# phtryll/subword-tokenizers

Hardware: AMD Instinct MI355X
Metric: FastBPE encode MB/s (value; tokens bit-exact) + BPE train s/1k-merges (train.s_per_1k_merges) (higher is better)
Workload: dtype u32; 1 GPU; configs[1]: FastBPE encode, S85k-open stand-in for train-85k (85,000 sentences, 8.53 MB/GPU), first 8,000 pretrained merges -- the slower of S85k-lex / S85k-open; sentences_per_gpu=85000, bytes_per_gpu=8526871, parallelism=corpus-sharded x1, no collective

## Files before the change

subword-tokenizers_amd/_build.py:

```python
import hashlib
import os
import shutil
import subprocess

_HERE = os.path.dirname(os.path.abspath(__file__))
CSRC = os.path.join(_HERE, "csrc")
LIB_DIR = os.path.join(_HERE, "_lib")
LIB_PATH = os.path.join(LIB_DIR, "libswt_hip.so")
SOURCES = ["swt_core.hip", "swt_tile.hip", "swt_dedup.hip", "swt_bpe_encode.hip", "swt_wp.hip", "swt_words.hip", "swt_bpe_train.hip", "swt_dist.hip", "swt_lower.hip", "swt_metrics.hip"]
HEADERS = ["swt_common.h", "swt_tile.h", "swt_dedup.h", "swt_words.h", "swt_train.h", "unicode_classes.inc", "unicode_lower.inc", os.path.join("..", "..", "include", "swt.h")]
FLAGS = ["--offload-arch=gfx950", "-O3", "-std=c++17", "-fPIC", "-Wall", "-Wno-unused-function"]
FLAGS += os.environ.get("SWT_EXTRA_FLAGS", "").split()


def _hipcc():
    for cand in (os.environ.get("HIPCC"), shutil.which("hipcc"), "/opt/rocm/bin/hipcc"):
        if cand and os.path.exists(cand):
            return cand
    raise RuntimeError("hipcc not found: libswt_hip.so cannot be built (set HIPCC or install ROCm)")


def _stamp():
    h = hashlib.sha256()
    for f in SOURCES + HEADERS:
        with open(os.path.join(CSRC, f), "rb") as fh:
            h.update(fh.read())
    h.update(" ".join(FLAGS).encode())
    return h.hexdigest()


def build(force=False, verbose=False):
    os.makedirs(LIB_DIR, exist_ok=True)
    stamp_path = os.path.join(LIB_DIR, "build.stamp")
    stamp = _stamp()
    if not force and os.path.exists(LIB_PATH) and os.path.exists(stamp_path):
        with open(stamp_path) as f:
            if f.read().strip() == stamp:
                return LIB_PATH
    hipcc = _hipcc()
    objs = []
    procs = []
    for src in SOURCES:
        obj = os.path.join(LIB_DIR, src.replace(".hip", ".o"))
        objs.append(obj)
        cmd = [hipcc] + FLAGS + ["-c", os.path.join(CSRC, src), "-o", obj]
        if verbose:
            print(" ".join(cmd))
        procs.append((src, subprocess.Popen(cmd, stdout=subprocess.PIPE, stderr=subprocess.STDOUT, text=True)))
    for src, p in procs:
        out, _ = p.communicate()
        if p.returncode != 0:
            raise RuntimeError("hipcc failed on %s:\n%s" % (src, out))
        if verbose and out.strip():
            print(out)
    cmd = [hipcc, "--offload-arch=gfx950", "-shared", "-fPIC", "-o", LIB_PATH] + objs + ["-ldl"]
    r = subprocess.run(cmd, stdout=subprocess.PIPE, stderr=subprocess.STDOUT, text=True)
    if r.returncode != 0:
        raise RuntimeError("link failed:\n" + r.stdout)
    with open(stamp_path, "w") as f:
        f.write(stamp)
    return LIB_PATH


# ... 31 lines not shown
```

subword-tokenizers_amd/csrc/swt_bpe_encode.hip:

```cpp
#include <cstring>
#include <unordered_map>
#include <utility>

#include "swt_dedup.h"
#include "swt_tile.h"
#include "swt_words.h"

namespace swt {

struct alignas(16) BpeSlot {
  uint64_t key;
  uint32_t rank;
  uint32_t merged;
};

constexpr uint8_t kClsWs = 1, kClsPunct = 2;
constexpr uint32_t kNoRank = 0xFFFFFFFFu;
#ifndef SWT_LANE_TILE
#define SWT_LANE_TILE 384
#endif
#ifndef SWT_LANE_CAP
#define SWT_LANE_CAP 512
#endif
constexpr int kLaneTile = SWT_LANE_TILE;
constexpr int kLaneCap = SWT_LANE_CAP;
constexpr uint64_t kDirectBytes = 1024, kDirectSents = 64;

struct BpeHash { uint32_t a, b, c; };
constexpr BpeHash kHash1{0x9E3779u, 0x85EBCBu, 0xC2B2AFu}, kHash2{0x27D4EBu, 0x165667u, 0x9E3779u};
__host__ __device__ __forceinline__ uint32_t bpe_hash(uint32_t l, uint32_t r, uint32_t sh, BpeHash k) {
  uint32_t x = (l & 0xFFFFFFu) * k.a + (r & 0xFFFFFFu) * k.b;
  x ^= x >> 16;
  return ((x & 0xFFFFFFu) * k.c) >> sh;
}

__device__ __forceinline__ bool slot_lookup(const BpeSlot *__restrict__ slots, uint32_t sh, uint32_t l, uint32_t r,
                                            uint32_t &rank, uint32_t &merged) {
  const uint4 r1 = *reinterpret_cast<const uint4 *>(&slots[bpe_hash(l, r, sh, kHash1)]);
  const uint4 r2 = *reinterpret_cast<const uint4 *>(&slots[bpe_hash(l, r, sh, kHash2)]);
  const bool h1 = r1.x == r && r1.y == l, h2 = r2.x == r && r2.y == l;
  rank = h1 ? r1.z : r2.z;
  merged = h1 ? r1.w : r2.w;
  return h1 || h2;
}

__device__ __forceinline__ uint32_t slot_value(const BpeSlot *__restrict__ slots, uint32_t sh, uint32_t l, uint32_t r) {
  const uint4 r1 = *reinterpret_cast<const uint4 *>(&slots[bpe_hash(l, r, sh, kHash1)]);
  const uint4 r2 = *reinterpret_cast<const uint4 *>(&slots[bpe_hash(l, r, sh, kHash2)]);
  const uint32_t a = (r1.x == r && r1.y == l) ? r1.z : kNoRank;
  const uint32_t b = (r2.x == r && r2.y == l) ? r2.z : kNoRank;
  return a & b;
}

__device__ uint32_t merge_word(uint32_t *s, uint32_t n, const BpeSlot *__restrict__ slots, uint32_t sh) {
  while (n >= 2) {
    uint32_t best = 0xFFFFFFFFu, bm = 0, bl = 0, br = 0;
    uint32_t a = s[0];
    for (uint32_t i = 0; i + 1 < n; i++) {
      const uint32_t b = s[i + 1];
      uint32_t rk, mg;
      if (slot_lookup(slots, sh, a, b, rk, mg) && rk < best) { best = rk; bm = mg; bl = a; br = b; }
      a = b;
    }
    if (best == 0xFFFFFFFFu) break;
    uint32_t j = 0, i = 0;
    while (i < n) {
      const uint32_t x = s[i];
      if (i + 1 < n && x == bl && s[i + 1] == br) { s[j++] = bm; i += 2; }
      else { s[j++] = x; i++; }
    }
    n = j;
  }
  return n;
}

struct GiantResult { uint64_t end; uint32_t ntok; };

__device__ GiantResult giant_word(const uint8_t *__restrict__ text, uint64_t pos, uint64_t send,
                                  const uint8_t *__restrict__ cls_tab, const BpeSlot *__restrict__ slots, uint32_t sh,
                                  uint32_t *out) {
  GiantResult r{pos, 0};
  uint32_t n = 0;
  bool first = true;
  while (r.end < send) {
    const uint8_t b = text[r.end];
    int len = utf8_len(b);
    if (r.end + len > send) len = (int)(send - r.end);
    uint32_t cp = b;
    if (b >= 0x80 && len > 1) {
      cp = b & (0xFF >> (len + 1));
      for (int i = 1; i < len; i++) cp = (cp << 6) | (text[r.end + i] & 0x3F);
    }
    const uint8_t c = utf8_is_cont(b) ? kClsWs : ((cls_tab && cp < kNumCodePoints) ? cls_tab[cp] : (uint8_t)0);
    if (c & kClsWs) { if (first) r.end += len; break; }
    if (c & kClsPunct) { if (first) { out[n++] = cp; r.end += len; } break; }
    out[n++] = cp;
    r.end += len;
    first = false;
  }
  n = merge_word(out, n, slots, sh);
  for (uint32_t i = 1; i < n; i++) out[i] |= SWT_BPE_CONT;
  r.ntok = n;
  return r;
}

template <int Cap>
struct LaneLds {
  static constexpr int Blocks = Cap / 64;
  __attribute__((aligned(16))) uint8_t txt[Cap + 16];
  uint32_t sym[Cap + 4];
  uint32_t val[Cap + 4];
  uint16_t wl[Cap + 2];
  unsigned long long sbits[Blocks + 1];
  unsigned long long symmask[Blocks + 1];
  unsigned long long vmask[Blocks + 1];
  uint32_t sympre[Blocks + 1];
  uint32_t blkpre[Blocks + 1];
};
struct LaneShared {
  uint32_t cls2[64];
  GiantResult giant;
};

struct LaneTile {
  uint64_t s_lo, s_hi;
  uint64_t span_base, span_end;
  uint64_t s_next;
  uint64_t cb;
  uint32_t *tile_out;
  uint32_t run;
};
struct LaneChunk {
  uint64_t abase;
  uint32_t off0, staged, nblk;
  uint32_t ce;
  uint32_t nsym, nw;
  int cut;
  bool last, giant;
};

__device__ __forceinline__ void wave_sync() {
  __builtin_amdgcn_fence(__ATOMIC_RELEASE, "wavefront");
  __builtin_amdgcn_wave_barrier();
  __builtin_amdgcn_fence(__ATOMIC_ACQUIRE, "wavefront");
}

constexpr uint32_t kDirtyVal = 0xFFFFFFFEu;

template <bool Packed>
__device__ void slow_word(uint32_t *S, uint32_t *V, const uint32_t n0, const BpeSlot *__restrict__ slots, uint32_t sh,
                          const uint32_t *__restrict__ merged_of_rank) {
  uint32_t n = n0;
  for (;;) {
    uint32_t m = kNoRank;
    for (uint32_t i = 0; i + 1 < n; i++) m = min(m, V[i]);
    if (m == kNoRank) break;
    const uint32_t mg = Packed ? (SWT_SYM_BASE + (m & 0xFFFFu)) : merged_of_rank[m];
    uint32_t i = 0, j = 0;
    while (i < n) {
      const uint32_t vi = V[i];
      const bool take = i + 1 < n && vi == m;
      const uint32_t s = take ? mg : (S[i] & ~SWT_BPE_CONT);
      if (take && j) V[j - 1] = kDirtyVal;
      S[j] = j ? (s | SWT_BPE_CONT) : s;
      V[j] = take ? kDirtyVal : vi;
      i += take ? 2u : 1u;
      j++;
    }
    n = j;
    V[n - 1] = kNoRank;
    for (uint32_t k = 0; k + 1 < n; k++)
      if (V[k] == kDirtyVal) V[k] = slot_value(slots, sh, S[k] & ~SWT_BPE_CONT, S[k + 1] & ~SWT_BPE_CONT);
  }
  for (uint32_t k = n; k < n0; k++) S[k] = kInvalidTok;
}

__device__ __forceinline__ void lane_classes(LaneShared &L, const uint8_t *__restrict__ cls_tab, int lane) {
  uint32_t w = 0;
  if (cls_tab) {
    const uint4 v = reinterpret_cast<const uint4 *>(cls_tab)[lane];
    auto pk = [](uint32_t d) {
      uint32_t x = d & 0x03030303u;
      x = (x | (x >> 6)) & 0x000F000Fu;
      return (x | (x >> 12)) & 0xFFu;
    };
    w = pk(v.x) | (pk(v.y) << 8) | (pk(v.z) << 16) | (pk(v.w) << 24);
  }
  L.cls2[lane] = w;
}

template <int Cap>
__device__ __forceinline__ void lane_split(LaneLds<Cap> &L, const uint32_t *cls2, const uint8_t *__restrict__ text, uint64_t n_bytes,
                                           const uint64_t *__restrict__ sent_off, const uint8_t *__restrict__ cls_tab,
                                           const BpeSlot *__restrict__ slots, uint32_t sh, const LaneTile &T, LaneChunk &C, int lane) {
  constexpr int Blocks = Cap / 64;
  const unsigned long long lt = (1ull << lane) - 1ull;
  const unsigned long long le = (2ull << lane) - 1ull;
  const uint64_t abase = T.cb & ~15ull;
  const uint32_t off0 = (uint32_t)(T.cb - abase);
  const uint64_t avail = T.span_end - abase;
  const bool last = avail <= (uint64_t)Cap;
  const uint32_t staged = last ? (uint32_t)avail : (uint32_t)Cap;
  const uint32_t nblk = (staged + 63) >> 6;

  for (uint32_t c = lane * 16; c < staged; c += 64 * 16) {
    const uint64_t g = abase + c;
    if (g + 16 <= n_bytes && ((reinterpret_cast<uintptr_t>(text + g) & 15) == 0)) {
      *reinterpret_cast<uint4 *>(&L.txt[c]) = *reinterpret_cast<const uint4 *>(text + g);
    } else {
      for (int i = 0; i < 16; i++) L.txt[c + i] = (g + i < n_bytes) ? text[g + i] : (uint8_t)' ';
    }
  }
  if (lane <= Blocks) L.sbits[lane] = 0ull;
  wave_sync();
  for (uint64_t s = T.s_next + lane; s < T.s_hi; s += 64) {
    const uint64_t o = sent_off[s];
    if (o >= abase + staged) break;
    if (o >= T.cb) atomicOr(&L.sbits[(o - abase) >> 6], 1ull << ((o - abase) & 63));
  }
  wave_sync();

  uint32_t nsym = 0, nw = 0;
  bool prev_wb = true;
  bool pend_open = false;
  uint32_t pend_cp = 0;
  int cut = -1;
  for (uint32_t blk = 0; blk < nblk; blk++) {
    const uint32_t p = blk * 64 + lane;
    const bool inr = p >= off0 && p < staged;
    const uint8_t b = inr ? L.txt[p] : (uint8_t)' ';
    const bool lead = !utf8_is_cont(b);
    uint32_t cp = b;
    if (b >= 0xC0) {
      int len = utf8_len(b);
      if (p + len > staged) len = (int)(staged - p);
      if (len > 1) {
        cp = b & (0xFF >> (len + 1));
        for (int i = 1; i < len; i++) cp = (cp << 6) | (L.txt[p + i] & 0x3F);
      }
    }
    uint32_t c = kClsWs;
    if (inr && lead)
      c = cp < 1024u ? ((cls2[cp >> 4] >> ((cp & 15u) << 1)) & 3u) : ((cls_tab && cp < kNumCodePoints) ? (cls_tab[cp] & 3u) : 0u);
    const unsigned long long INR = __ballot(inr);
    const unsigned long long LEAD = __ballot(lead);
    const unsigned long long WSm = __ballot(lead && (c & kClsWs));
    const unsigned long long PNm = __ballot(lead && (c & kClsPunct));
    const unsigned long long CONT = ~LEAD;
    unsigned long long WB = WSm | PNm | ((prev_wb && (CONT & 1ull)) ? 1ull : 0ull);
    WB |= (WB << 1) & CONT;
    WB |= (WB << 1) & CONT;
    WB |= (WB << 1) & CONT;
    const unsigned long long SS = L.sbits[blk];
    const unsigned long long first_bit = blk == 0 ? (1ull << off0) : 0ull;
    const unsigned long long before = (WB << 1) | (prev_wb ? 1ull : 0ull) | SS | first_bit;
    const unsigned long long SYM = LEAD & ~WSm & INR;
    const unsigned long long WSTART = SYM & (PNm | before);
    {
      const unsigned long long CUT = LEAD & (WSm | PNm | SS) & __ballot(inr && p > off0 && p + 4 <= staged);
      if (CUT) cut = (int)(blk * 64 + 63 - __builtin_clzll(CUT));
    }
    const bool is_sym = (SYM >> lane) & 1ull;
    const bool wstart = (WSTART >> lane) & 1ull;
    const unsigned long long after = SYM & ~le;
    const uint32_t q = after ? (uint32_t)__builtin_ctzll(after) : 64u;
    const bool hasnext = is_sym && q < 64 && !((WSTART >> (q & 63)) & 1ull);
    const uint32_t f = SYM ? (uint32_t)__builtin_ctzll(SYM) : 64u;
    const bool joins = pend_open && f < 64 && !((WSTART >> (f & 63)) & 1ull);
    const uint32_t si = nsym + (uint32_t)__popcll(SYM & lt);
    const uint32_t cpn = __shfl(cp, (int)(q & 63));
    const bool jp = joins && lane == 63;
    const uint32_t cpf = __builtin_amdgcn_readlane(cp, (int)(f & 63));
    const bool want = hasnext || jp;
    uint32_t v = kNoRank;
    if (want) v = slot_value(slots, sh, jp ? pend_cp : cp, jp ? cpf : cpn);
    if (is_sym) {
      L.sym[si] = wstart ? cp : (cp | SWT_BPE_CONT);
      if (!hasnext) L.val[si] = kNoRank;
    }
    if (want) L.val[jp ? nsym - 1 : si] = v;
    if (wstart) L.wl[nw + (uint32_t)__popcll(WSTART & lt)] = (uint16_t)si;
    if (lane == 0) { L.symmask[blk] = SYM; L.sympre[blk] = nsym; }
    nw += (uint32_t)__popcll(WSTART);
    nsym += (uint32_t)__popcll(SYM);
    if (SYM) {
      const int li = 63 - __builtin_clzll(SYM);
      const unsigned long long tail = li == 63 ? 0ull : ~((2ull << li) - 1ull);
      pend_open = ((WSm | PNm | SS) & tail) == 0ull && !((PNm >> li) & 1ull);
      pend_cp = __builtin_amdgcn_readlane(cp, li);
    } else {
      pend_open = false;
    }
    prev_wb = (WB >> 63) & 1ull;
  }
  wave_sync();
  C.abase = abase;
  C.off0 = off0;
  C.staged = staged;
  C.nblk = nblk;
  C.ce = staged;
  C.nsym = nsym;
  C.nw = nw;
  C.cut = cut;
  C.last = last;
  C.giant = false;
}

template <int Cap, int Mode>
__device__ __forceinline__ void lane_chunk_end(LaneLds<Cap> &L, GiantResult &giant, const uint8_t *__restrict__ text, const uint64_t *__restrict__ sent_off,
                                               const uint8_t *__restrict__ cls_tab, const BpeSlot *__restrict__ slots, uint32_t sh,
                                               LaneTile &T, LaneChunk &C, int lane, uint32_t *__restrict__ sent_local,
                                               const uint32_t *__restrict__ uslot, unsigned long long *__restrict__ rec,
                                               unsigned long long *__restrict__ drec, const DirectOut &direct) {
  constexpr bool kDirect = Mode == 2, kRec = Mode == 1;
  if (!C.last) {
    if (C.cut < 0) {
      if (lane == 0) {
        uint64_t s = T.s_next;
        while (s < T.s_hi && sent_off[s] <= T.cb) s++;
        const uint64_t send = sent_off[s];
        giant = giant_word(text, T.cb, send, cls_tab, slots, sh, T.tile_out + T.run);
      }
      wave_sync();
      const GiantResult g = giant;
      uint32_t mine = 0;
      for (uint64_t s = T.s_next + lane; s < T.s_hi; s += 64) {
        if (sent_off[s] >= g.end) break;
        if (kDirect) direct.off[s] = T.run; else if (Mode == 0) sent_local[s] = T.run;
        if (kRec) {
          drec[s] = (unsigned long long)(T.span_base + T.run) | ((unsigned long long)g.ntok << 32);
          rec[uslot[s]] = (unsigned long long)s | ((unsigned long long)g.ntok << 32);
        }
        mine++;
      }
      for (int d = 32; d >= 1; d >>= 1) mine += __shfl_xor(mine, d);
      T.s_next += mine;
      T.run += g.ntok;
      T.cb = g.end;
      C.giant = true;
      C.nw = 0;
      C.nsym = 0;
      wave_sync();
      return;
    }
    C.ce = (uint32_t)C.cut;
    C.nsym = L.sympre[C.ce >> 6] + (uint32_t)__popcll(L.symmask[C.ce >> 6] & ((1ull << (C.ce & 63)) - 1ull));
    uint32_t keep = 0;
    for (uint32_t k0 = 0; k0 < C.nw; k0 += 64) {
      const uint32_t k = k0 + lane;
      keep += (uint32_t)__popcll(__ballot(k < C.nw && L.wl[k] < C.nsym));
    }
    C.nw = keep;
  }
  if (lane == 0) L.wl[C.nw] = (uint16_t)C.nsym;
  T.cb = C.abase + C.ce;
  wave_sync();
}

template <int Cap>
__device__ __forceinline__ void lane_words_count(const LaneLds<Cap> &L, uint32_t nw, int lane, uint32_t &c2, uint32_t &c1, uint32_t &c0) {
  c0 = c1 = c2 = 0;
  for (uint32_t k0 = 0; k0 < nw; k0 += 64) {
    const uint32_t k = k0 + lane;
    const uint32_t n = k < nw ? (uint32_t)L.wl[k + 1] - (uint32_t)L.wl[k] : 0u;
    c0 += (uint32_t)__popcll(__ballot(n >= 2 && n <= 4));
    c1 += (uint32_t)__popcll(__ballot(n >= 5 && n <= 8));
    c2 += (uint32_t)__popcll(__ballot(n >= 9));
  }
}
template <int Cap>
__device__ __forceinline__ void lane_words_write(const LaneLds<Cap> &L, uint32_t nw, int lane, uint16_t *list, uint32_t o2, uint32_t o1,
                                                 uint32_t o0) {
  const unsigned long long lt = (1ull << lane) - 1ull;
  for (uint32_t k0 = 0; k0 < nw; k0 += 64) {
    const uint32_t k = k0 + lane;
    const uint32_t n = k < nw ? (uint32_t)L.wl[k + 1] - (uint32_t)L.wl[k] : 0u;
    const unsigned long long M0 = __ballot(n >= 2 && n <= 4), M1 = __ballot(n >= 5 && n <= 8), M2 = __ballot(n >= 9);
    if (n >= 9) list[o2 + (uint32_t)__popcll(M2 & lt)] = (uint16_t)k;
    else if (n >= 5) list[o1 + (uint32_t)__popcll(M1 & lt)] = (uint16_t)k;
    else if (n >= 2) list[o0 + (uint32_t)__popcll(M0 & lt)] = (uint16_t)k;
    o0 += (uint32_t)__popcll(M0);
    o1 += (uint32_t)__popcll(M1);
    o2 += (uint32_t)__popcll(M2);
  }
}

template <bool Packed>
__device__ __forceinline__ uint32_t rank_key(uint32_t v, uint32_t slot) {
  return Packed ? ((v & 0xFFFF0000u) | slot) : (v >= (1u << 27) ? (0xFFFFFFE0u | slot) : ((v << 5) | slot));
}
template <bool Packed>
__device__ __forceinline__ uint32_t scan_key(const uint32_t *V, uint32_t n) {
  const uint32_t nm1 = n - 1u;
  uint32_t key = 0xFFFFFFFFu;
  for (uint32_t i0 = 0; i0 < nm1; i0 += 4) {
    const uint32_t i1 = min(i0 + 1u, nm1), i2 = min(i0 + 2u, nm1), i3 = min(i0 + 3u, nm1);
    const uint32_t k0 = rank_key<Packed>(V[i0], i0), k1 = rank_key<Packed>(V[i1], i1);
    const uint32_t k2 = rank_key<Packed>(V[i2], i2), k3 = rank_key<Packed>(V[i3], i3);
    key = min(min(key, k0), min(min(k1, k2), k3));
  }
  return key;
}
struct LaneWord {
  uint32_t n, alive;
  uint32_t where;
// ... 580 lines not shown
```

subword-tokenizers_amd/csrc/swt_dedup.hip:

```cpp

#include "swt_dedup.h"

namespace swt {

constexpr uint8_t kClsWs = SWT_CLS_BERT_WS, kClsPunct = SWT_CLS_BERT_PUNCT, kClsPySpace = SWT_CLS_PY_SPACE;
constexpr int kClsLds = 1024;
#ifndef SWT_DTILE
#define SWT_DTILE 1024
#endif
#ifndef SWT_DCAP
#define SWT_DCAP 1536
#endif
constexpr int kDTile = SWT_DTILE;
constexpr int kDCap = SWT_DCAP;
constexpr int kDBlocks = kDCap / 64;
#ifndef SWT_WORDREF_WAVES
#define SWT_WORDREF_WAVES 7
#endif
constexpr unsigned long long kDOffMask = (1ull << 40) - 1ull;
constexpr uint32_t kRefSlot = 0x80000000u;

typedef uint64_t u64u __attribute__((aligned(1)));

struct DedupTab {
  unsigned long long *slot;
  unsigned long long *rec;
  uint64_t n_bytes;
  uint32_t bits;
  uint32_t epoch;
  uint32_t ovf_shift;
  unsigned long long *newlist;
  unsigned long long *tile_new;
};

constexpr uint32_t kDdMaxProbes = 24;
__device__ __forceinline__ uint32_t dd_own_slot(const DedupTab &D, uint64_t gpos) { return (1u << D.bits) + (uint32_t)(gpos >> D.ovf_shift); }

__device__ __forceinline__ unsigned long long dd_pack8(const uint8_t *p, uint32_t n) {
  unsigned long long w = 0;
  for (uint32_t i = 0; i < n && i < 8; i++) w |= (unsigned long long)p[i] << (8 * i);
  return w;
}
__device__ __forceinline__ unsigned long long dd_hash(const uint8_t *p, uint32_t n) {
  const unsigned long long w0 = dd_pack8(p, n), w1 = n > 8 ? dd_pack8(p + 8, n - 8) : 0ull;
  unsigned long long h = (w0 ^ 0x9E3779B97F4A7C15ull) * 0xff51afd7ed558ccdull;
  h ^= h >> 32;
  h = (h ^ w1 ^ ((unsigned long long)n << 56)) * 0xc4ceb9fe1a85ec53ull;
  for (uint32_t i = 16; i < n; i += 8) {
    h ^= h >> 29;
    h = (h ^ dd_pack8(p + i, n - i)) * 0x9E3779B97F4A7C15ull;
  }
  h ^= h >> 29; h *= 0x94d049bb133111ebull; h ^= h >> 32;
  return h;
}

__device__ uint32_t dd_find_or_insert(const DedupTab &D, const uint8_t *__restrict__ text, const uint8_t *mine, uint32_t len,
                                      uint64_t gpos, bool &is_new) {
  is_new = false;
  if (len >= 255u) { is_new = true; return dd_own_slot(D, gpos); }
// ... 52 lines not shown
  for (int p = 0; p < 2; p++) {
    const unsigned long long v = D.slot[j];
    if ((v & ~kDOffMask) == head) {
      const uint64_t ro = v & kDOffMask;
      if (ro + 16 <= D.n_bytes) {
        const uint8_t *rep = text + ro;
        unsigned long long r0 = *reinterpret_cast<const u64u *>(rep), r1 = *reinterpret_cast<const u64u *>(rep + 8);
        if (len < 8) { r0 &= (1ull << (8 * len)) - 1ull; r1 = 0; }
        else if (len < 16) r1 &= (1ull << (8 * (len - 8))) - 1ull;
        bool same = r0 == w0 && r1 == w1;
        for (uint32_t i = 16; i < len && same; i++) same = rep[i] == mine[i];
        if (same) return j;
      } else {
        break;
      }
    } else if ((uint32_t)(v >> 56) != D.epoch) {
      break;
    }
    j = (j + 1) & mask;
  }
  for (;;) {
    unsigned long long v = __hip_atomic_load(&D.slot[idx], __ATOMIC_RELAXED, __HIP_MEMORY_SCOPE_AGENT);
    if ((uint32_t)(v >> 56) != D.epoch) {
      const unsigned long long prev = atomicCAS(&D.slot[idx], v, head | gpos);
      if (prev == v) {
        is_new = true;
        return idx;
      }
      v = prev;
      if ((uint32_t)(v >> 56) != D.epoch) continue;
    }
    if ((v & ~kDOffMask) == head) {
      const uint64_t ro = v & kDOffMask;
      const uint8_t *rep = text + ro;
      bool same;
      if (ro + 16 <= D.n_bytes) {
        unsigned long long r0 = *reinterpret_cast<const u64u *>(rep), r1 = *reinterpret_cast<const u64u *>(rep + 8);
        if (len < 8) { r0 &= (1ull << (8 * len)) - 1ull; r1 = 0; }
        else if (len < 16) r1 &= (1ull << (8 * (len - 8))) - 1ull;
        same = r0 == w0 && r1 == w1;
        for (uint32_t i = 16; i < len && same; i++) same = rep[i] == mine[i];
      } else {
        same = true;
        for (uint32_t i = 0; i < len; i++)
          if (rep[i] != mine[i]) { same = false; break; }
      }
      if (same) return idx;
    }
    if (++probes >= kDdMaxProbes) { is_new = true; return dd_own_slot(D, gpos); }
    idx = (idx + 1) & mask;
  }
}

__device__ __forceinline__ uint32_t dd_nibble(uint32_t flags_bit7) {
  return ((((flags_bit7 >> 7) & 0x01010101u) * 0x01020408u) >> 24) & 0xFu;
}

struct WordrefLds {
  __attribute__((aligned(16))) uint8_t txt[kDCap + 16];
  uint16_t wl[kDCap];
  unsigned long long sbits[kDBlocks + 1];
  unsigned long long endm[kDBlocks + 1];
  uint32_t cls2[kClsLds / 16];
  unsigned long long wst[kDBlocks + 1];
  uint32_t nwb[kDBlocks + 1];
  uint64_t giant_end;
  uint32_t giant_new, giant_word;
};

template <int Mode>
__global__ __launch_bounds__(64, SWT_WORDREF_WAVES) void wordref_kernel(const uint8_t *__restrict__ text, uint64_t n_bytes,
                                                     const uint64_t *__restrict__ sent_off, const uint64_t *__restrict__ plan,
                                                     const uint8_t *__restrict__ cls_tab, DedupTab D, uint32_t *__restrict__ wref,
                                                     uint32_t *__restrict__ sent_word, uint32_t *__restrict__ tile_words) {
  constexpr uint8_t kWsBit = Mode == kDedupWp ? kClsPySpace : kClsWs;
  constexpr bool kPunctSplits = Mode == kDedupBpe;
  __shared__ WordrefLds L;
  const int lane = threadIdx.x;
  const unsigned long long lt = (1ull << lane) - 1ull;
  const uint64_t t = blockIdx.x;
  const uint64_t s_lo = plan[t], s_hi = plan[t + 1];
  if (s_lo == s_hi) {
    if (lane == 0) { D.tile_new[t] = 0ull; tile_words[t] = 0u; }
    return;
  }
  {
    const uint4 v = reinterpret_cast<const uint4 *>(cls_tab)[lane];
    auto pk = [](uint32_t d) {
      uint32_t ws = d & (0x01010101u * kWsBit), pn = kPunctSplits ? (d & (0x01010101u * kClsPunct)) : 0u;
      ws = ws / kWsBit;
      pn = (pn / kClsPunct) << 1;
      uint32_t x = ws | pn;
      x = (x | (x >> 6)) & 0x000F000Fu;
      return (x | (x >> 12)) & 0xFFu;
    };
    L.cls2[lane] = pk(v.x) | (pk(v.y) << 8) | (pk(v.z) << 16) | (pk(v.w) << 24);
  }
  const uint64_t span_base = sent_off[s_lo], span_end = sent_off[s_hi];
  uint64_t s_next = s_lo;
  uint64_t cb = span_base;
  unsigned long long *const my_list = D.newlist + (Mode == kDedupWp ? span_base : (span_base >> 1));
  uint32_t *const my_rec = wref + span_base;
  uint32_t n_new = 0, words_done = 0;
  unsigned long long my_bytes = 0;
  for (;;) {
    const uint64_t abase = cb & ~15ull;
    const uint32_t off0 = (uint32_t)(cb - abase);
    const uint64_t avail = span_end - abase;
    const bool last = avail <= (uint64_t)kDCap;
    const uint32_t staged = last ? (uint32_t)avail : (uint32_t)kDCap;
    const uint32_t nblk = (staged + 63) >> 6;
    for (uint32_t c = lane * 16; c < staged; c += 64 * 16) {
      const uint64_t g = abase + c;
      if (g + 16 <= n_bytes && ((reinterpret_cast<uintptr_t>(text + g) & 15) == 0)) {
        *reinterpret_cast<uint4 *>(&L.txt[c]) = *reinterpret_cast<const uint4 *>(text + g);
      } else {
        for (int i = 0; i < 16; i++) L.txt[c + i] = (g + i < n_bytes) ? text[g + i] : (uint8_t)' ';
      }
    }
    if (lane <= kDBlocks) L.sbits[lane] = 0ull;
    __syncthreads();
    for (uint64_t s = s_next + lane; s < s_hi; s += 64) {
      const uint64_t o = sent_off[s];
      if (o >= abase + staged) break;
      if (o >= cb) atomicOr(&L.sbits[(o - abase) >> 6], 1ull << ((o - abase) & 63));
    }
    __syncthreads();
    uint32_t nw = 0;
    int cut = -1;
    uint32_t carry_wb = 0x8000u, carry_ct = 0u;
    const uint32_t n_groups = nblk * 4;
    for (uint32_t g0 = 0; g0 < n_groups; g0 += 64) {
      const uint32_t g = g0 + (uint32_t)lane, p0 = g * 16;
      const uint4 x = *reinterpret_cast<const uint4 *>(&L.txt[p0 < (uint32_t)kDCap ? p0 : 0]);
      uint32_t sp_all = 0, pn_all = 0, ct_all = 0, hi_all = 0;
#pragma unroll
      for (int q = 0; q < 4; q++) {
        const uint32_t w = q == 0 ? x.x : (q == 1 ? x.y : (q == 2 ? x.z : x.w)), x7 = w & 0x7F7F7F7Fu, hi = w & 0x80808080u;
#define SWT_IN(lo_, hi_) ((x7 + (0x80u - (lo_)) * 0x01010101u) & ~(x7 + (0x7Fu - (hi_)) * 0x01010101u))
        uint32_t in_ws, in_pn = 0;
        if (Mode == kDedupWp) {
          in_ws = SWT_IN(0x09u, 0x0Du) | SWT_IN(0x1Cu, 0x20u);
        } else {
          in_ws = SWT_IN(0x09u, 0x0Du) | SWT_IN(0x20u, 0x20u);
          in_pn = SWT_IN(0x21u, 0x2Fu) | SWT_IN(0x3Au, 0x40u) | SWT_IN(0x5Bu, 0x60u) | SWT_IN(0x7Bu, 0x7Eu);
        }
#undef SWT_IN
        sp_all |= dd_nibble(in_ws & ~hi & 0x80808080u) << (4 * q);
        if (kPunctSplits) pn_all |= dd_nibble(in_pn & ~hi & 0x80808080u) << (4 * q);
        ct_all |= dd_nibble(hi & ~(w << 1)) << (4 * q);
        hi_all |= dd_nibble(hi & (w << 1)) << (4 * q);
      }
      const uint32_t lo = off0 > p0 ? (off0 - p0 < 16u ? off0 - p0 : 16u) : 0u;
      const uint32_t hi_n = staged > p0 ? (staged - p0 < 16u ? staged - p0 : 16u) : 0u;
      const uint32_t inr16 = (((1u << hi_n) - 1u) & ~((1u << lo) - 1u)) & 0xFFFFu;
      uint32_t sp16 = sp_all & inr16, pn16 = pn_all & inr16;
      const uint32_t ct16 = ct_all & inr16;
      for (uint32_t m = hi_all & inr16; m; m &= m - 1u) {
        const uint32_t j = (uint32_t)__builtin_ctz(m), p = p0 + j;
        const uint8_t b = L.txt[p];
        int len = utf8_len(b);
        if (p + len > staged) len = (int)(staged - p);
        uint32_t cp = b;
        if (len > 1) {
          cp = b & (0xFF >> (len + 1));
          for (int i = 1; i < len; i++) cp = (cp << 6) | (L.txt[p + i] & 0x3F);
        }
        uint32_t c2;
        if (cp < (uint32_t)kClsLds) {
          c2 = (L.cls2[cp >> 4] >> ((cp & 15u) << 1)) & 3u;
        } else {
          const uint8_t c = cp < kNumCodePoints ? cls_tab[cp] : (uint8_t)0;
          c2 = ((c & kWsBit) ? 1u : 0u) | ((kPunctSplits && (c & kClsPunct)) ? 2u : 0u);
        }
        if (c2 & 1u) sp16 |= 1u << j;
        if (c2 & 2u) pn16 |= 1u << j;
      }
      const uint32_t wsm16 = (sp16 | ~inr16) & 0xFFFFu;
      const uint32_t lead16 = ~ct16 & 0xFFFFu;
      const uint32_t raw16 = wsm16 | pn16;
      uint32_t below_wb = __shfl_up(raw16, 1), below_ct = __shfl_up(ct16, 1);
      if (lane == 0) { below_wb = carry_wb; below_ct = carry_ct; }
      const uint32_t c32 = below_ct | (ct16 << 16);
      uint32_t wb32 = below_wb | (raw16 << 16);
      wb32 |= (wb32 << 1) & c32;
      wb32 |= (wb32 << 1) & c32;
      wb32 |= (wb32 << 1) & c32;
      const uint32_t ss16 = reinterpret_cast<const uint16_t *>(L.sbits)[g < (uint32_t)(kDBlocks + 1) * 4u ? g : 0];
      const uint32_t first16 = g == 0 ? (1u << off0) : 0u;
      const uint32_t before16 = ((wb32 >> 15) | ss16 | first16) & 0xFFFFu;
      const uint32_t sym16 = lead16 & ~wsm16 & inr16;
      const uint32_t ws16 = sym16 & (pn16 | before16);
      const uint32_t c_lo = off0 + 1u > p0 ? (off0 + 1u - p0 < 16u ? off0 + 1u - p0 : 16u) : 0u;
      const uint32_t c_hi = staged >= p0 + 4u ? (staged - 3u - p0 < 16u ? staged - 3u - p0 : 16u) : 0u;
      const uint32_t cutr16 = (c_hi > c_lo ? (((1u << c_hi) - 1u) & ~((1u << c_lo) - 1u)) : 0u) & 0xFFFFu;
      const uint32_t cut16 = lead16 & (wsm16 | pn16 | ss16) & cutr16 & inr16;
      const unsigned long long CUTL = __ballot(cut16 != 0u);
      if (CUTL) {
        const int src = 63 - __builtin_clzll(CUTL);
        const uint32_t top = __shfl(cut16, src);
        cut = (int)((g0 + (uint32_t)src) * 16u + 31u - (uint32_t)__builtin_clz(top));
      }
      const uint32_t n_mine = (uint32_t)__popc(ws16);
      uint32_t incl = n_mine;
      for (int d = 1; d < 64; d <<= 1) {
        const uint32_t y = __shfl_up(incl, d);
        if (lane >= d) incl += y;
      }
      uint32_t at = nw + incl - n_mine;
      if (g < n_groups) {
        reinterpret_cast<uint16_t *>(L.endm)[g] = (uint16_t)(wsm16 | ws16);
        reinterpret_cast<uint16_t *>(L.wst)[g] = (uint16_t)ws16;
        if ((g & 3u) == 0u) L.nwb[g >> 2] = at;
        for (uint32_t m = ws16; m; m &= m - 1u) L.wl[at++] = (uint16_t)(p0 + (uint32_t)__builtin_ctz(m));
      }
      nw += __shfl(incl, 63);
      carry_wb = __shfl(raw16, 63);
      carry_ct = __shfl(ct16, 63);
    }
    __syncthreads();
    uint32_t ce = staged;
    if (!last) {
      if (cut < 0) {
        if (lane == 0) {
          uint64_t s = s_next;
          while (s < s_hi && sent_off[s] <= cb) s++;
          const uint64_t send = sent_off[s];
          uint64_t e = cb;
          bool first = true, has_word = true;
          uint32_t nchar = 0, cp0 = 0;
          while (e < send) {
            const uint8_t b = text[e];
            int len = utf8_len(b);
            if (e + len > send) len = (int)(send - e);
            uint32_t cp = b;
            if (b >= 0x80 && len > 1) {
              cp = b & (0xFF >> (len + 1));
              for (int i = 1; i < len; i++) cp = (cp << 6) | (text[e + i] & 0x3F);
            }
            const uint8_t c = utf8_is_cont(b) ? kWsBit : (cp < kNumCodePoints ? cls_tab[cp] : (uint8_t)0);
            if (c & kWsBit) { if (first) { e += len; has_word = false; } break; }
            if (kPunctSplits && (c & kClsPunct)) { if (first) { e += len; nchar = 1; cp0 = cp; } break; }
            if (first) cp0 = cp;
            nchar++;
            e += len;
            first = false;
          }
          L.giant_new = 0;
          L.giant_word = 0;
          if (has_word && e > cb) {
            L.giant_word = 1;
            if (Mode == kDedupBpe && nchar == 1) {
              my_rec[words_done] = cp0;
            } else {
              bool fresh;
              const uint64_t wl = e - cb;
              const uint32_t idx = dd_find_or_insert(D, text, text + cb, (uint32_t)wl, cb, fresh);
              my_rec[words_done] = kRefSlot | idx;
              if (fresh) {
                D.rec[idx] = wl;
                my_list[n_new] = ((unsigned long long)idx << 32) | cb;
                my_bytes += wl;
                L.giant_new = 1;
              }
            }
          }
          L.giant_end = e;
        }
        __syncthreads();
        const uint32_t wd_before = words_done;
        cb = L.giant_end;
// ... 506 lines not shown
```

Measured before the change: 52380 MB/s.

## Reuse 16-byte-per-lane split classifier in BPE encode lane path and batch pair lookups

Moves the SWAR 16-bytes-per-lane word/symbol classification from the dedup kernel into a shared header and uses it in the BPE encode lane split. Previously the encode path processed 64 bytes per wave iteration with several ballots and a serial carry of pending-word state. It now computes symbol and word-start masks plus prefix counts for 1024 bytes per iteration, then scatters symbols, and finally computes adjacent-pair merge ranks in a separate pass that reads the symbol array. The word count at the cut is taken from prefix sums instead of a ballot loop. The cost is an extra pass over LDS and extra hash probes with predicated dummy loads, plus the risk of subtle boundary differences in carry handling (the carry is only propagated when Cap>1024).

```diff
diff --git a/subword-tokenizers_amd/_build.py b/subword-tokenizers_amd/_build.py
--- a/subword-tokenizers_amd/_build.py
+++ b/subword-tokenizers_amd/_build.py
@@ -8,7 +8,7 @@
 LIB_DIR = os.path.join(_HERE, "_lib")
 LIB_PATH = os.path.join(LIB_DIR, "libswt_hip.so")
 SOURCES = ["swt_core.hip", "swt_tile.hip", "swt_dedup.hip", "swt_bpe_encode.hip", "swt_wp.hip", "swt_words.hip", "swt_bpe_train.hip", "swt_dist.hip", "swt_lower.hip", "swt_metrics.hip"]
-HEADERS = ["swt_common.h", "swt_tile.h", "swt_dedup.h", "swt_words.h", "swt_train.h", "unicode_classes.inc", "unicode_lower.inc", os.path.join("..", "..", "include", "swt.h")]
+HEADERS = ["swt_common.h", "swt_tile.h", "swt_dedup.h", "swt_split16.h", "swt_words.h", "swt_train.h", "unicode_classes.inc", "unicode_lower.inc", os.path.join("..", "..", "include", "swt.h")]
 FLAGS = ["--offload-arch=gfx950", "-O3", "-std=c++17", "-fPIC", "-Wall", "-Wno-unused-function"]
 FLAGS += os.environ.get("SWT_EXTRA_FLAGS", "").split()
 
diff --git a/subword-tokenizers_amd/csrc/swt_bpe_encode.hip b/subword-tokenizers_amd/csrc/swt_bpe_encode.hip
--- a/subword-tokenizers_amd/csrc/swt_bpe_encode.hip
+++ b/subword-tokenizers_amd/csrc/swt_bpe_encode.hip
@@ -3,6 +3,7 @@
 #include <utility>
 
 #include "swt_dedup.h"
+#include "swt_split16.h"
 #include "swt_tile.h"
 #include "swt_words.h"
 
@@ -49,6 +50,15 @@
   const uint4 r2 = *reinterpret_cast<const uint4 *>(&slots[bpe_hash(l, r, sh, kHash2)]);
   const uint32_t a = (r1.x == r && r1.y == l) ? r1.z : kNoRank;
   const uint32_t b = (r2.x == r && r2.y == l) ? r2.z : kNoRank;
+  return a & b;
+}
+
+__device__ __forceinline__ uint32_t slot_value_if(const BpeSlot *__restrict__ slots, uint32_t sh, uint32_t l, uint32_t r, bool has) {
+  const uint32_t i1 = has ? bpe_hash(l, r, sh, kHash1) : 0u, i2 = has ? bpe_hash(l, r, sh, kHash2) : 0u;
+  const uint4 r1 = *reinterpret_cast<const uint4 *>(&slots[i1]);
+  const uint4 r2 = *reinterpret_cast<const uint4 *>(&slots[i2]);
+  const uint32_t a = (has && r1.x == r && r1.y == l) ? r1.z : kNoRank;
+  const uint32_t b = (has && r2.x == r && r2.y == l) ? r2.z : kNoRank;
   return a & b;
 }
 
@@ -113,9 +123,15 @@
   uint16_t wl[Cap + 2];
   unsigned long long sbits[Blocks + 1];
   unsigned long long symmask[Blocks + 1];
-  unsigned long long vmask[Blocks + 1];
+  union {
+    unsigned long long wst[Blocks + 1];
+    unsigned long long vmask[Blocks + 1];
+  };
   uint32_t sympre[Blocks + 1];
-  uint32_t blkpre[Blocks + 1];
+  union {
+    uint32_t wpre[Blocks + 1];
+    uint32_t blkpre[Blocks + 1];
+  };
 };
 struct LaneShared {
   uint32_t cls2[64];
@@ -195,7 +211,6 @@
                                            const BpeSlot *__restrict__ slots, uint32_t sh, const LaneTile &T, LaneChunk &C, int lane) {
   constexpr int Blocks = Cap / 64;
   const unsigned long long lt = (1ull << lane) - 1ull;
-  const unsigned long long le = (2ull << lane) - 1ull;
   const uint64_t abase = T.cb & ~15ull;
   const uint32_t off0 = (uint32_t)(T.cb - abase);
   const uint64_t avail = T.span_end - abase;
@@ -221,77 +236,65 @@
   wave_sync();
 
   uint32_t nsym = 0, nw = 0;
-  bool prev_wb = true;
-  bool pend_open = false;
-  uint32_t pend_cp = 0;
   int cut = -1;
+  uint32_t carry_wb = 0x8000u, carry_ct = 0u;
+  const uint32_t n_groups = nblk * 4;
+  for (uint32_t g0 = 0; g0 < n_groups; g0 += 64) {
+    const uint32_t g = g0 + (uint32_t)lane;
+    const Split16 m = split16<kClsWs, true>(L.txt, (uint32_t)Cap, cls2, cls_tab, cls_tab != nullptr, L.sbits, (uint32_t)(Blocks + 1) * 4u, g, off0,
+                                            staged, carry_wb, carry_ct, lane);
+    cut = split16_cut(m.cut16, g0, cut);
+    const uint32_t mine = (uint32_t)__popc(m.ws16) | ((uint32_t)__popc(m.sym16) << 16);
+    const uint32_t incl = split16_scan(mine, lane);
+    if (g < n_groups) {
+      reinterpret_cast<uint16_t *>(L.symmask)[g] = (uint16_t)m.sym16;
+      reinterpret_cast<uint16_t *>(L.wst)[g] = (uint16_t)m.ws16;
+      if ((g & 3u) == 0u) {
+        const uint32_t before = incl - mine;
+        L.wpre[g >> 2] = nw + (before & 0xFFFFu);
+        L.sympre[g >> 2] = nsym + (before >> 16);
+      }
+    }
+    const uint32_t all = __builtin_amdgcn_readlane(incl, 63);
+    nw += all & 0xFFFFu;
+    nsym += all >> 16;
+    if (Cap > 1024) {
+      carry_wb = __builtin_amdgcn_readlane(m.raw16, 63);
+      carry_ct = __builtin_amdgcn_readlane(m.ct16, 63);
+    }
+  }
+  wave_sync();
+
   for (uint32_t blk = 0; blk < nblk; blk++) {
-    const uint32_t p = blk * 64 + lane;
-    const bool inr = p >= off0 && p < staged;
-    const uint8_t b = inr ? L.txt[p] : (uint8_t)' ';
-    const bool lead = !utf8_is_cont(b);
-    uint32_t cp = b;
-    if (b >= 0xC0) {
-      int len = utf8_len(b);
-      if (p + len > staged) len = (int)(staged - p);
-      if (len > 1) {
-        cp = b & (0xFF >> (len + 1));
-        for (int i = 1; i < len; i++) cp = (cp << 6) | (L.txt[p + i] & 0x3F);
-      }
-    }
-    uint32_t c = kClsWs;
-    if (inr && lead)
-      c = cp < 1024u ? ((cls2[cp >> 4] >> ((cp & 15u) << 1)) & 3u) : ((cls_tab && cp < kNumCodePoints) ? (cls_tab[cp] & 3u) : 0u);
-    const unsigned long long INR = __ballot(inr);
-    const unsigned long long LEAD = __ballot(lead);
-    const unsigned long long WSm = __ballot(lead && (c & kClsWs));
-    const unsigned long long PNm = __ballot(lead && (c & kClsPunct));
-    const unsigned long long CONT = ~LEAD;
-    unsigned long long WB = WSm | PNm | ((prev_wb && (CONT & 1ull)) ? 1ull : 0ull);
-    WB |= (WB << 1) & CONT;
-    WB |= (WB << 1) & CONT;
-    WB |= (WB << 1) & CONT;
-    const unsigned long long SS = L.sbits[blk];
-    const unsigned long long first_bit = blk == 0 ? (1ull << off0) : 0ull;
-    const unsigned long long before = (WB << 1) | (prev_wb ? 1ull : 0ull) | SS | first_bit;
-    const unsigned long long SYM = LEAD & ~WSm & INR;
-    const unsigned long long WSTART = SYM & (PNm | before);
-    {
-      const unsigned long long CUT = LEAD & (WSm | PNm | SS) & __ballot(inr && p > off0 && p + 4 <= staged);
-      if (CUT) cut = (int)(blk * 64 + 63 - __builtin_clzll(CUT));
-    }
-    const bool is_sym = (SYM >> lane) & 1ull;
-    const bool wstart = (WSTART >> lane) & 1ull;
-    const unsigned long long after = SYM & ~le;
-    const uint32_t q = after ? (uint32_t)__builtin_ctzll(after) : 64u;
-    const bool hasnext = is_sym && q < 64 && !((WSTART >> (q & 63)) & 1ull);
-    const uint32_t f = SYM ? (uint32_t)__builtin_ctzll(SYM) : 64u;
-    const bool joins = pend_open && f < 64 && !((WSTART >> (f & 63)) & 1ull);
-    const uint32_t si = nsym + (uint32_t)__popcll(SYM & lt);
-    const uint32_t cpn = __shfl(cp, (int)(q & 63));
-    const bool jp = joins && lane == 63;
-    const uint32_t cpf = __builtin_amdgcn_readlane(cp, (int)(f & 63));
-    const bool want = hasnext || jp;
-    uint32_t v = kNoRank;
-    if (want) v = slot_value(slots, sh, jp ? pend_cp : cp, jp ? cpf : cpn);
-    if (is_sym) {
+    const unsigned long long SYM = L.symmask[blk], WST = L.wst[blk];
+    if ((SYM >> lane) & 1ull) {
+      const uint32_t p = blk * 64 + lane;
+      const uint8_t b = L.txt[p];
+      uint32_t cp = b;
+      if (b >= 0xC0) {
+        int len = utf8_len(b);
+        if (p + len > staged) len = (int)(staged - p);
+        if (len > 1) {
+          cp = b & (0xFF >> (len + 1));
+          for (int i = 1; i < len; i++) cp = (cp << 6) | (L.txt[p + i] & 0x3F);
+        }
+      }
+      const bool wstart = (WST >> lane) & 1ull;
+      const uint32_t si = L.sympre[blk] + (uint32_t)__popcll(SYM & lt);
       L.sym[si] = wstart ? cp : (cp | SWT_BPE_CONT);
-      if (!hasnext) L.val[si] = kNoRank;
-    }
-    if (want) L.val[jp ? nsym - 1 : si] = v;
-    if (wstart) L.wl[nw + (uint32_t)__popcll(WSTART & lt)] = (uint16_t)si;
-    if (lane == 0) { L.symmask[blk] = SYM; L.sympre[blk] = nsym; }
-    nw += (uint32_t)__popcll(WSTART);
-    nsym += (uint32_t)__popcll(SYM);
-    if (SYM) {
-      const int li = 63 - __builtin_clzll(SYM);
-      const unsigned long long tail = li == 63 ? 0ull : ~((2ull << li) - 1ull);
-      pend_open = ((WSm | PNm | SS) & tail) == 0ull && !((PNm >> li) & 1ull);
-      pend_cp = __builtin_amdgcn_readlane(cp, li);
-    } else {
-      pend_open = false;
-    }
-    prev_wb = (WB >> 63) & 1ull;
+      if (wstart) L.wl[L.wpre[blk] + (uint32_t)__popcll(WST & lt)] = (uint16_t)si;
+    }
+  }
+  if (lane == 0) L.sym[nsym] = 0u;
+  wave_sync();
+  for (uint32_t j0 = 0; j0 < nsym; j0 += 128) {
+    const uint32_t ja = j0 + (uint32_t)lane, jb = ja + 64u;
+    const uint32_t ia = min(ja, nsym), ib = min(jb, nsym);
+    const uint32_t a0 = L.sym[ia], a1 = L.sym[ia + 1u], b0 = L.sym[ib], b1 = L.sym[ib + 1u];
+    const uint32_t va = slot_value_if(slots, sh, a0 & ~SWT_BPE_CONT, a1 & ~SWT_BPE_CONT, ja < nsym && (a1 & SWT_BPE_CONT));
+    const uint32_t vb = slot_value_if(slots, sh, b0 & ~SWT_BPE_CONT, b1 & ~SWT_BPE_CONT, jb < nsym && (b1 & SWT_BPE_CONT));
+    if (ja < nsym) L.val[ja] = va;
+    if (jb < nsym) L.val[jb] = vb;
   }
   wave_sync();
   C.abase = abase;
@@ -345,12 +348,7 @@
     }
     C.ce = (uint32_t)C.cut;
     C.nsym = L.sympre[C.ce >> 6] + (uint32_t)__popcll(L.symmask[C.ce >> 6] & ((1ull << (C.ce & 63)) - 1ull));
-    uint32_t keep = 0;
-    for (uint32_t k0 = 0; k0 < C.nw; k0 += 64) {
-      const uint32_t k = k0 + lane;
-      keep += (uint32_t)__popcll(__ballot(k < C.nw && L.wl[k] < C.nsym));
-    }
-    C.nw = keep;
+    C.nw = L.wpre[C.ce >> 6] + (uint32_t)__popcll(L.wst[C.ce >> 6] & ((1ull << (C.ce & 63)) - 1ull));
   }
   if (lane == 0) L.wl[C.nw] = (uint16_t)C.nsym;
   T.cb = C.abase + C.ce;
diff --git a/subword-tokenizers_amd/csrc/swt_dedup.hip b/subword-tokenizers_amd/csrc/swt_dedup.hip
--- a/subword-tokenizers_amd/csrc/swt_dedup.hip
+++ b/subword-tokenizers_amd/csrc/swt_dedup.hip
@@ -1,10 +1,11 @@
 
 #include "swt_dedup.h"
+#include "swt_split16.h"
 
 namespace swt {
 
 constexpr uint8_t kClsWs = SWT_CLS_BERT_WS, kClsPunct = SWT_CLS_BERT_PUNCT, kClsPySpace = SWT_CLS_PY_SPACE;
-constexpr int kClsLds = 1024;
+constexpr int kClsLds = (int)kSplitClsLds;
 #ifndef SWT_DTILE
 #define SWT_DTILE 1024
 #endif
@@ -163,10 +164,6 @@
   }
 }
 
-__device__ __forceinline__ uint32_t dd_nibble(uint32_t flags_bit7) {
-  return ((((flags_bit7 >> 7) & 0x01010101u) * 0x01020408u) >> 24) & 0xFu;
-}
-
 struct WordrefLds {
   __attribute__((aligned(16))) uint8_t txt[kDCap + 16];
   uint16_t wl[kDCap];
@@ -243,81 +240,12 @@
     const uint32_t n_groups = nblk * 4;
     for (uint32_t g0 = 0; g0 < n_groups; g0 += 64) {
       const uint32_t g = g0 + (uint32_t)lane, p0 = g * 16;
-      const uint4 x = *reinterpret_cast<const uint4 *>(&L.txt[p0 < (uint32_t)kDCap ? p0 : 0]);
-      uint32_t sp_all = 0, pn_all = 0, ct_all = 0, hi_all = 0;
-#pragma unroll
-      for (int q = 0; q < 4; q++) {
-        const uint32_t w = q == 0 ? x.x : (q == 1 ? x.y : (q == 2 ? x.z : x.w)), x7 = w & 0x7F7F7F7Fu, hi = w & 0x80808080u;
-#define SWT_IN(lo_, hi_) ((x7 + (0x80u - (lo_)) * 0x01010101u) & ~(x7 + (0x7Fu - (hi_)) * 0x01010101u))
-        uint32_t in_ws, in_pn = 0;
-        if (Mode == kDedupWp) {
-          in_ws = SWT_IN(0x09u, 0x0Du) | SWT_IN(0x1Cu, 0x20u);
-        } else {
-          in_ws = SWT_IN(0x09u, 0x0Du) | SWT_IN(0x20u, 0x20u);
-          in_pn = SWT_IN(0x21u, 0x2Fu) | SWT_IN(0x3Au, 0x40u) | SWT_IN(0x5Bu, 0x60u) | SWT_IN(0x7Bu, 0x7Eu);
-        }
-#undef SWT_IN
-        sp_all |= dd_nibble(in_ws & ~hi & 0x80808080u) << (4 * q);
-        if (kPunctSplits) pn_all |= dd_nibble(in_pn & ~hi & 0x80808080u) << (4 * q);
-        ct_all |= dd_nibble(hi & ~(w << 1)) << (4 * q);
-        hi_all |= dd_nibble(hi & (w << 1)) << (4 * q);
-      }
-      const uint32_t lo = off0 > p0 ? (off0 - p0 < 16u ? off0 - p0 : 16u) : 0u;
-      const uint32_t hi_n = staged > p0 ? (staged - p0 < 16u ? staged - p0 : 16u) : 0u;
-      const uint32_t inr16 = (((1u << hi_n) - 1u) & ~((1u << lo) - 1u)) & 0xFFFFu;
-      uint32_t sp16 = sp_all & inr16, pn16 = pn_all & inr16;
-      const uint32_t ct16 = ct_all & inr16;
-      for (uint32_t m = hi_all & inr16; m; m &= m - 1u) {
-        const uint32_t j = (uint32_t)__builtin_ctz(m), p = p0 + j;
-        const uint8_t b = L.txt[p];
-        int len = utf8_len(b);
-        if (p + len > staged) len = (int)(staged - p);
-        uint32_t cp = b;
-        if (len > 1) {
-          cp = b & (0xFF >> (len + 1));
-          for (int i = 1; i < len; i++) cp = (cp << 6) | (L.txt[p + i] & 0x3F);
-        }
-        uint32_t c2;
-        if (cp < (uint32_t)kClsLds) {
-          c2 = (L.cls2[cp >> 4] >> ((cp & 15u) << 1)) & 3u;
-        } else {
-          const uint8_t c = cp < kNumCodePoints ? cls_tab[cp] : (uint8_t)0;
-          c2 = ((c & kWsBit) ? 1u : 0u) | ((kPunctSplits && (c & kClsPunct)) ? 2u : 0u);
-        }
-        if (c2 & 1u) sp16 |= 1u << j;
-        if (c2 & 2u) pn16 |= 1u << j;
-      }
-      const uint32_t wsm16 = (sp16 | ~inr16) & 0xFFFFu;
-      const uint32_t lead16 = ~ct16 & 0xFFFFu;
-      const uint32_t raw16 = wsm16 | pn16;
-      uint32_t below_wb = __shfl_up(raw16, 1), below_ct = __shfl_up(ct16, 1);
-      if (lane == 0) { below_wb = carry_wb; below_ct = carry_ct; }
-      const uint32_t c32 = below_ct | (ct16 << 16);
-      uint32_t wb32 = below_wb | (raw16 << 16);
-      wb32 |= (wb32 << 1) & c32;
-      wb32 |= (wb32 << 1) & c32;
-      wb32 |= (wb32 << 1) & c32;
-      const uint32_t ss16 = reinterpret_cast<const uint16_t *>(L.sbits)[g < (uint32_t)(kDBlocks + 1) * 4u ? g : 0];
-      const uint32_t first16 = g == 0 ? (1u << off0) : 0u;
-      const uint32_t before16 = ((wb32 >> 15) | ss16 | first16) & 0xFFFFu;
-      const uint32_t sym16 = lead16 & ~wsm16 & inr16;
-      const uint32_t ws16 = sym16 & (pn16 | before16);
-      const uint32_t c_lo = off0 + 1u > p0 ? (off0 + 1u - p0 < 16u ? off0 + 1u - p0 : 16u) : 0u;
-      const uint32_t c_hi = staged >= p0 + 4u ? (staged - 3u - p0 < 16u ? staged - 3u - p0 : 16u) : 0u;
-      const uint32_t cutr16 = (c_hi > c_lo ? (((1u << c_hi) - 1u) & ~((1u << c_lo) - 1u)) : 0u) & 0xFFFFu;
-      const uint32_t cut16 = lead16 & (wsm16 | pn16 | ss16) & cutr16 & inr16;
-      const unsigned long long CUTL = __ballot(cut16 != 0u);
-      if (CUTL) {
-        const int src = 63 - __builtin_clzll(CUTL);
-        const uint32_t top = __shfl(cut16, src);
-        cut = (int)((g0 + (uint32_t)src) * 16u + 31u - (uint32_t)__builtin_clz(top));
-      }
+      const Split16 m16 = split16<kWsBit, kPunctSplits>(L.txt, (uint32_t)kDCap, L.cls2, cls_tab, true, L.sbits, (uint32_t)(kDBlocks + 1) * 4u, g,
+                                                        off0, staged, carry_wb, carry_ct, lane);
+      const uint32_t wsm16 = m16.wsm16, ws16 = m16.ws16;
+      cut = split16_cut(m16.cut16, g0, cut);
       const uint32_t n_mine = (uint32_t)__popc(ws16);
-      uint32_t incl = n_mine;
-      for (int d = 1; d < 64; d <<= 1) {
-        const uint32_t y = __shfl_up(incl, d);
-        if (lane >= d) incl += y;
-      }
+      const uint32_t incl = split16_scan(n_mine, lane);
       uint32_t at = nw + incl - n_mine;
       if (g < n_groups) {
         reinterpret_cast<uint16_t *>(L.endm)[g] = (uint16_t)(wsm16 | ws16);
@@ -326,8 +254,8 @@
         for (uint32_t m = ws16; m; m &= m - 1u) L.wl[at++] = (uint16_t)(p0 + (uint32_t)__builtin_ctz(m));
       }
       nw += __shfl(incl, 63);
-      carry_wb = __shfl(raw16, 63);
-      carry_ct = __shfl(ct16, 63);
+      carry_wb = __shfl(m16.raw16, 63);
+      carry_ct = __shfl(m16.ct16, 63);
     }
     __syncthreads();
     uint32_t ce = staged;
diff --git a/subword-tokenizers_amd/csrc/swt_split16.h b/subword-tokenizers_amd/csrc/swt_split16.h
--- /dev/null
+++ b/subword-tokenizers_amd/csrc/swt_split16.h
@@ -0,0 +1,114 @@
+#pragma once
+#include "swt_common.h"
+
+namespace swt {
+
+constexpr uint32_t kSplitClsLds = 1024;
+
+__device__ __forceinline__ uint32_t split16_nibble(uint32_t flags_bit7) {
+  return ((((flags_bit7 >> 7) & 0x01010101u) * 0x01020408u) >> 24) & 0xFu;
+}
+
+struct Split16 {
+  uint32_t raw16;
+  uint32_t ct16;
+  uint32_t wsm16;
+  uint32_t ss16;
+  uint32_t sym16;
+  uint32_t ws16;
+  uint32_t cut16;
+};
+
+template <uint32_t kWsBit, bool kPunctSplits>
+__device__ __forceinline__ Split16 split16(const uint8_t *txt, uint32_t txt_cap, const uint32_t *cls2, const uint8_t *__restrict__ cls_tab,
+                                           bool classes, const unsigned long long *sbits, uint32_t sbits_groups, uint32_t g, uint32_t off0,
+                                           uint32_t staged, uint32_t below0_wb, uint32_t below0_ct, int lane) {
+  const uint32_t p0 = g * 16;
+  const uint4 x = *reinterpret_cast<const uint4 *>(&txt[p0 < txt_cap ? p0 : 0]);
+  uint32_t sp_all = 0, pn_all = 0, ct_all = 0, hi_all = 0;
+#pragma unroll
+  for (int q = 0; q < 4; q++) {
+    const uint32_t w = q == 0 ? x.x : (q == 1 ? x.y : (q == 2 ? x.z : x.w)), x7 = w & 0x7F7F7F7Fu, hi = w & 0x80808080u;
+#define SWT_IN(lo_, hi_) ((x7 + (0x80u - (lo_)) * 0x01010101u) & ~(x7 + (0x7Fu - (hi_)) * 0x01010101u))
+    uint32_t in_ws, in_pn = 0;
+    if (kWsBit == SWT_CLS_PY_SPACE) {
+      in_ws = SWT_IN(0x09u, 0x0Du) | SWT_IN(0x1Cu, 0x20u);
+    } else {
+      in_ws = SWT_IN(0x09u, 0x0Du) | SWT_IN(0x20u, 0x20u);
+    }
+    if (kPunctSplits) in_pn = SWT_IN(0x21u, 0x2Fu) | SWT_IN(0x3Au, 0x40u) | SWT_IN(0x5Bu, 0x60u) | SWT_IN(0x7Bu, 0x7Eu);
+#undef SWT_IN
+    sp_all |= split16_nibble(in_ws & ~hi & 0x80808080u) << (4 * q);
+    if (kPunctSplits) pn_all |= split16_nibble(in_pn & ~hi & 0x80808080u) << (4 * q);
+    ct_all |= split16_nibble(hi & ~(w << 1)) << (4 * q);
+    hi_all |= split16_nibble(hi & (w << 1)) << (4 * q);
+  }
+  if (!classes) sp_all = pn_all = hi_all = 0u;
+  const uint32_t lo = off0 > p0 ? (off0 - p0 < 16u ? off0 - p0 : 16u) : 0u;
+  const uint32_t hi_n = staged > p0 ? (staged - p0 < 16u ? staged - p0 : 16u) : 0u;
+  const uint32_t inr16 = (((1u << hi_n) - 1u) & ~((1u << lo) - 1u)) & 0xFFFFu;
+  uint32_t sp16 = sp_all & inr16, pn16 = pn_all & inr16;
+  const uint32_t ct16 = ct_all & inr16;
+  for (uint32_t m = hi_all & inr16; m; m &= m - 1u) {
+    const uint32_t j = (uint32_t)__builtin_ctz(m), p = p0 + j;
+    const uint8_t b = txt[p];
+    int len = utf8_len(b);
+    if (p + len > staged) len = (int)(staged - p);
+    uint32_t cp = b;
+    if (len > 1) {
+      cp = b & (0xFF >> (len + 1));
+      for (int i = 1; i < len; i++) cp = (cp << 6) | (txt[p + i] & 0x3F);
+    }
+    uint32_t c2;
+    if (cp < kSplitClsLds) {
+      c2 = (cls2[cp >> 4] >> ((cp & 15u) << 1)) & 3u;
+    } else {
+      const uint8_t c = cp < kNumCodePoints ? cls_tab[cp] : (uint8_t)0;
+      c2 = ((c & kWsBit) ? 1u : 0u) | ((kPunctSplits && (c & SWT_CLS_BERT_PUNCT)) ? 2u : 0u);
+    }
+    if (c2 & 1u) sp16 |= 1u << j;
+    if (c2 & 2u) pn16 |= 1u << j;
+  }
+  Split16 r;
+  r.wsm16 = (sp16 | ~inr16) & 0xFFFFu;
+  r.ct16 = ct16;
+  const uint32_t lead16 = ~ct16 & 0xFFFFu;
+  r.raw16 = r.wsm16 | pn16;
+  uint32_t below_wb = __shfl_up(r.raw16, 1), below_ct = __shfl_up(ct16, 1);
+  if (lane == 0) { below_wb = below0_wb; below_ct = below0_ct; }
+  const uint32_t c32 = below_ct | (ct16 << 16);
+  uint32_t wb32 = below_wb | (r.raw16 << 16);
+  wb32 |= (wb32 << 1) & c32;
+  wb32 |= (wb32 << 1) & c32;
+  wb32 |= (wb32 << 1) & c32;
+  r.ss16 = reinterpret_cast<const uint16_t *>(sbits)[g < sbits_groups ? g : 0];
+  const uint32_t first16 = g == 0 ? (1u << off0) : 0u;
+  const uint32_t before16 = ((wb32 >> 15) | r.ss16 | first16) & 0xFFFFu;
+  r.sym16 = lead16 & ~r.wsm16 & inr16;
+  r.ws16 = r.sym16 & (pn16 | before16);
+  const uint32_t c_lo = off0 + 1u > p0 ? (off0 + 1u - p0 < 16u ? off0 + 1u - p0 : 16u) : 0u;
+  const uint32_t c_hi = staged >= p0 + 4u ? (staged - 3u - p0 < 16u ? staged - 3u - p0 : 16u) : 0u;
+  const uint32_t cutr16 = (c_hi > c_lo ? (((1u << c_hi) - 1u) & ~((1u << c_lo) - 1u)) : 0u) & 0xFFFFu;
+  r.cut16 = lead16 & (r.wsm16 | pn16 | r.ss16) & cutr16 & inr16;
+  return r;
+}
+
+__device__ __forceinline__ int split16_cut(uint32_t cut16, uint32_t g0, int cut) {
+  const unsigned long long CUTL = __ballot(cut16 != 0u);
+  if (CUTL) {
+    const int src = 63 - __builtin_clzll(CUTL);
+    const uint32_t top = __builtin_amdgcn_readlane(cut16, src);
+    cut = (int)((g0 + (uint32_t)src) * 16u + 31u - (uint32_t)__builtin_clz(top));
+  }
+  return cut;
+}
+
+__device__ __forceinline__ uint32_t split16_scan(uint32_t v, int lane) {
+  for (int d = 1; d < 64; d <<= 1) {
+    const uint32_t y = __shfl_up(v, d);
+    if (lane >= d) v += y;
+  }
+  return v;
+}
+
+}
```

Result: no change. 52590 MB/s, median of 6 (+0.4%).
